# NVIDIA/flowtron

Measured on NVIDIA B200. Metric: training mel-frames/sec, higher is better.
Workload: dtype f16 tensor-core operands (loss-scaled in backward), f32 accumulate+state

## Files before the change

### flowtron_b200/_lib.py

```python
from __future__ import annotations

import ctypes
import os
from ctypes import POINTER, Structure, byref, c_char_p, c_double, c_float, c_int, c_longlong, c_size_t, c_void_p

import torch

_HERE = os.path.dirname(os.path.abspath(__file__))
LIB_PATH = os.path.join(_HERE, "libflowtron_b200.so")

FT_F16, FT_BF16, FT_TF32 = 0, 1, 2
_FMT = {torch.float16: FT_F16, torch.bfloat16: FT_BF16, torch.float32: FT_TF32}

_lib = None


class FtArStepDesc(Structure):
    _fields_ = [("T", c_int), ("B", c_int), ("L", c_int), ("n_mel", c_int), ("n_hidden", c_int), ("n_attn", c_int),
                ("n_text", c_int), ("reversed", c_int), ("has_gate", c_int), ("has_prior", c_int),
                ("temperature", c_float)]


AR_WEIGHT_FIELDS = ["attn_lstm_w_ih", "attn_lstm_w_hh", "attn_lstm_b_ih", "attn_lstm_b_hh",
                    "lstm_w_ih0", "lstm_w_hh0", "lstm_b_ih0", "lstm_b_hh0",
# ... 166 lines not shown


def timing_report():
    buf = ctypes.create_string_buffer(1 << 16)
    lib().ft_timing_report.argtypes = [c_char_p, c_int]
    n = lib().ft_timing_report(buf, len(buf))
    out = []
    for line in buf.raw[:n].decode().splitlines():
        name, m, nn, k, cnt, ms = line.split()
        out.append((name, int(m), int(nn), int(k), int(cnt), float(ms)))
    return out


def _need_cuda(*ts):
    for t in ts:
        if t is not None and not t.is_cuda:
            raise FlowtronB200Error("flowtron_b200 kernels need CUDA tensors (no CPU fallback exists)")


def set_gemm_pair_mode(mode: int):
    lib().ft_set_gemm_pair_mode(int(mode))


def gemm(A, B, *, a_mn=False, b_mn=False, bias=None, bias2=None, act=0, beta=0, alpha=1.0,
         out32=None, out16=None):
    _need_cuda(A, B)
    if a_mn:
        K, M = A.shape
    else:
        M, K = A.shape
    if b_mn:
        Kb, N = B.shape
    else:
        N, Kb = B.shape
    assert K == Kb, (A.shape, B.shape)
    assert A.stride(-1) == 1 and B.stride(-1) == 1
    c16_fmt = 0
    if out16 is not None:
        c16_fmt = _FMT[out16.dtype]
    check(lib().ft_gemm(M, N, K, ptr(A), A.stride(0), _FMT[A.dtype], int(a_mn), ptr(B), B.stride(0), _FMT[B.dtype],
                        int(b_mn), ptr(bias), ptr(bias2), act, beta, float(alpha),
                        ptr(out32), 0 if out32 is None else out32.stride(0),
                        ptr(out16), 0 if out16 is None else out16.stride(0), c16_fmt, stream_ptr()), "ft_gemm")


def lstm_fwd(xproj, whh16, lens, hseq16, gates16=None, cstate=None, h32=None):
# ... 251 lines not shown
```

### flowtron_b200/csrc/api.cu

```cuda
#include <mutex>
#include <string>
#include <atomic>
#include <cstdio>
#include <vector>
#include <map>
#include <tuple>

#include "ft_internal.h"
#include "../../include/flowtron_b200.h"

namespace ft {

static thread_local std::string g_err;
static std::atomic<long long> g_launches{0};
static int* g_status_dev = nullptr;
static std::mutex g_mu;

int ft_set_error(const char* msg) {
    g_err = msg ? msg : "unknown error";
    return -1;
}
int ft_check_launch(const char* what) {
    cudaError_t e = cudaGetLastError();
    if (e != cudaSuccess) {
// ... 75 lines not shown
    }
    return off;
}

long long ft_launch_count(void) { return ft::g_launches.load(); }
void ft_reset_launch_count(void) { ft::g_launches.store(0); }

int ft_gemm(int M, int N, int K, const void* A, long long lda, int a_fmt, int a_mn, const void* B, long long ldb,
            int b_fmt, int b_mn, const float* bias, const float* bias2, int act, int beta, float alpha, float* C32,
            long long ldc32, void* C16, long long ldc16, int c16_fmt, void* stream) {
    ft::GemmArgs g;
    g.M = M; g.N = N; g.K = K;
    g.A = A; g.lda = lda; g.a_fmt = a_fmt; g.a_mn = a_mn;
    g.B = B; g.ldb = ldb; g.b_fmt = b_fmt; g.b_mn = b_mn;
    g.bias = bias; g.bias2 = bias2; g.act = act; g.beta = beta; g.alpha = alpha;
    g.C32 = C32; g.ldc32 = ldc32; g.C16 = C16; g.ldc16 = ldc16; g.c16_fmt = c16_fmt;
    return ft::launch_gemm(g, static_cast<cudaStream_t>(stream));
}

void ft_debug_set_lstm_trace(long long* buf) { ft::set_lstm_trace(buf); }

void ft_set_lstm_half_sm(int on) { ft::set_lstm_half_sm(on); }
void ft_set_gemm_pair_mode(int mode) { ft::set_gemm_pair_mode(mode); }

int ft_lstm_fwd(int T, int B, const float* xproj, const void* whh16, const int* lens, void* hseq16, long long ldh,
                void* gates16, float* cstate, float* h32, long long ldh32, int* flags, void* stream) {
    return ft::launch_lstm_fwd(T, B, xproj, whh16, lens, hseq16, ldh, gates16, cstate, h32, ldh32, flags,
                               static_cast<cudaStream_t>(stream));
}

int ft_lstm_bwd(int T, int B, const float* dh_ext, long long ldd, const void* whhT16, const void* gates16,
                const float* cstate, const int* lens, void* dG16, int* flags, void* stream) {
    return ft::launch_lstm_bwd(T, B, dh_ext, ldd, whhT16, gates16, cstate, lens, dG16, flags,
                               static_cast<cudaStream_t>(stream));
}

}
```

### flowtron_b200/csrc/ar_step.cu

```cuda
#include <cstdlib>
#include <cstring>
#include <map>
#include <mutex>
#include <string>
#include <vector>

#include "ft_internal.h"
#include "../../include/flowtron_b200.h"

namespace ft {

namespace {

constexpr int H = 1024, G = 4096;

struct Region { const char* name; size_t off, bytes; };

struct Plan {
    uint8_t* base = nullptr;
    size_t off = 0;
    std::vector<Region>* regs = nullptr;
    template <typename T>
    T* get(const char* name, size_t n) {
        const size_t bytes = n * sizeof(T);
// ... 220 lines not shown
static Pipe* get_pipe(cudaStream_t main) {
    std::lock_guard<std::mutex> lk(g_side_mu);
    auto it = g_pipes.find(main);
    if (it != g_pipes.end()) return &it->second;
    Pipe pp;
    int prio_lo = 0, prio_hi = 0;
    cudaDeviceGetStreamPriorityRange(&prio_lo, &prio_hi);
    const int pr = pipe_prio() ? prio_hi : prio_lo;
    if (cudaStreamCreateWithPriority(&pp.sA, cudaStreamNonBlocking, pr) != cudaSuccess) return nullptr;
    if (cudaStreamCreateWithPriority(&pp.sB, cudaStreamNonBlocking, pr) != cudaSuccess) return nullptr;
    const int mid = pipe_prio() && prio_hi < prio_lo - 1 ? prio_lo - 1 : prio_lo;
    if (cudaStreamCreateWithPriority(&pp.sC, cudaStreamNonBlocking, mid) != cudaSuccess) return nullptr;
    if (cudaStreamCreateWithPriority(&pp.sD, cudaStreamNonBlocking, prio_lo) != cudaSuccess) return nullptr;
    cudaEventCreateWithFlags(&pp.evJ, cudaEventDisableTiming);
    cudaEventCreateWithFlags(&pp.evD, cudaEventDisableTiming);
    cudaEventCreateWithFlags(&pp.evA, cudaEventDisableTiming);
    cudaEventCreateWithFlags(&pp.evG, cudaEventDisableTiming);
    cudaEventCreateWithFlags(&pp.evB, cudaEventDisableTiming);
    cudaEventCreateWithFlags(&pp.ev0, cudaEventDisableTiming);
    g_pipes[main] = pp;
    return &g_pipes[main];
}

int zero(void* p, size_t bytes, cudaStream_t st) {
    return cudaMemsetAsync(p, 0, bytes, st) == cudaSuccess ? 0 : ft_set_error("cudaMemsetAsync failed");
}
int copy_f32(float* dst, const float* src, size_t n, cudaStream_t st) {
    return cudaMemcpyAsync(dst, src, n * sizeof(float), cudaMemcpyDeviceToDevice, st) == cudaSuccess ? 0 : ft_set_error("cudaMemcpyAsync failed");
}

}

static thread_local cudaEvent_t g_text_ready = nullptr;
void set_text_ready_event(void* ev) { g_text_ready = static_cast<cudaEvent_t>(ev); }

int ar_step_fwd(const FtArStepDesc& d, const FtArStepWeights& w, const float* mel, const float* text, const int* in_lens,
                const int* out_lens, const float* prior, float* mel_out, float* log_s, float* gates, float* attn,
                float* logprob, void* saved, void* scratch, cudaStream_t st) {
    cudaEvent_t text_ready = g_text_ready;
    g_text_ready = nullptr;
    FT_TRY(check_desc(d));
    if (d.has_prior && !prior) return ft_set_error("ar_step_fwd: has_prior set but attn_prior is NULL");
    if (d.has_gate && (!gates || !w.gate_w)) return ft_set_error("ar_step_fwd: has_gate set but gate pointers are NULL");
    const Dims n(d);
    Plan ps; ps.base = static_cast<uint8_t*>(saved);
    Saved S; S.plan(ps, d);
// ... 37 lines not shown
    auto kv_projections = [&](cudaStream_t s2) -> int {
        if (text_ready) {
            if (cudaStreamWaitEvent(s2, text_ready, 0) != cudaSuccess) return ft_set_error("ar_step_fwd: cudaStreamWaitEvent(text_ready) failed");
        }
        FT_TRY(launch_cast(text, 2, S.text16, 0, n.RL * n.E, s2));
        FT_TRY(gemm_fwd(s2, n.RL, n.A, n.E, S.text16, n.E, F.w.wk, n.E, nullptr, nullptr, 0, S.Kp, n.A, nullptr, 0));
        FT_TRY(gemm_fwd(s2, n.RL, n.A, n.E, S.text16, n.E, F.w.wv, n.E, nullptr, nullptr, 0, S.Vp, n.A, nullptr, 0));
        return 0;
    };
    if (pa) {
        const int CH = att_chunk;
        auto xa = [&](cudaStream_t s2, int t0, int t1) {
            const long long r0 = static_cast<long long>(t0) * n.B, rows = static_cast<long long>(t1 - t0) * n.B;
            return gemm_fwd(s2, rows, G, n.M, S.mel_in16 + r0 * n.M, n.M, F.w.w_ih_a, n.M, w.attn_lstm_b_ih, w.attn_lstm_b_hh, 0,
                            F.X1 + r0 * G, G, nullptr, 0);
        };
        cudaStream_t sr = pipe_prio() ? pa->sA : st;
        cudaEventRecord(pa->ev0, st);
        if (sr != st) cudaStreamWaitEvent(sr, pa->ev0, 0);
        cudaStreamWaitEvent(pa->sB, pa->ev0, 0);
        cudaStreamWaitEvent(pa->sC, pa->ev0, 0);
        FT_TRY(kv_projections(pa->sC));
        FT_TRY(xa(sr, 0, CH < n.T ? CH : n.T));
        for (int t0 = 0; t0 < n.T; t0 += CH) {
            const int t1 = t0 + CH < n.T ? t0 + CH : n.T;
            if (t1 < n.T) {
                FT_TRY(xa(pa->sB, t1, t1 + CH < n.T ? t1 + CH : n.T));
                cudaEventRecord(pa->evB, pa->sB);
            }
            FT_TRY(launch_lstm_fwd_chunk(n.T, n.B, t0, t1, F.X1, F.w.w_hh_a, out_lens, S.d16, n.D, S.gatesA, S.cA, F.flags, sr, F.hA32, H));
            cudaEventRecord(pa->evA, sr);
            if (t1 < n.T) cudaStreamWaitEvent(sr, pa->evB, 0);
            cudaStreamWaitEvent(pa->sC, pa->evA, 0);
            FT_TRY(attention_rows(pa->sC, t0, t1));
            const long long r0 = static_cast<long long>(t0) * n.B, rows = static_cast<long long>(t1 - t0) * n.B;
            FT_TRY(gemm_fwd(pa->sC, rows, G, n.D, S.d16 + r0 * n.D, n.D, F.w.w_ih0, n.D, w.lstm_b_ih0, w.lstm_b_hh0, 0, F.X + r0 * G, G, nullptr, 0));
        }
        cudaEventRecord(pa->evG, pa->sC);
        cudaStreamWaitEvent(st, pa->evG, 0);
        if (sr != st) { cudaEventRecord(pa->evJ, sr); cudaStreamWaitEvent(st, pa->evJ, 0); }
        xproj0_done = true;
    } else {
    static int xin = -1;
    if (xin < 0) { const char* e = getenv("FT_LSTM_XIN"); xin = (!e || atoi(e) != 0) ? 1 : 0; }
    if (xin && n.M <= 128 && n.B <= 32) {
        FT_TRY(launch_lstm_fwd_xin(n.T, n.B, S.mel_in16, n.M, n.M, F.w.w_ih_a, w.attn_lstm_b_ih, w.attn_lstm_b_hh, F.w.w_hh_a, out_lens,
                                   S.d16, n.D, S.gatesA, S.cA, F.hA32, H, F.flags, st));
    } else {
        FT_TRY(gemm_fwd(st, n.R, G, n.M, S.mel_in16, n.M, F.w.w_ih_a, n.M, w.attn_lstm_b_ih, w.attn_lstm_b_hh, 0, F.X, G, nullptr, 0));
        FT_TRY(launch_lstm_fwd(n.T, n.B, F.X, F.w.w_hh_a, out_lens, S.d16, n.D, S.gatesA, S.cA, F.hA32, H, F.flags, st));
    }
    FT_TRY(kv_projections(st));
    FT_TRY(attention_rows(st, 0, n.T));
    }

    Pipe* pp = (F.X1 && n.B <= 32 && n.T > pipe_chunk_steps()) ? get_pipe(st) : nullptr;
    if (pp) {
        const int S_ = pipe_chunk_steps();
        int* flagsA = F.flags;
        int* flagsB = F.flags + static_cast<size_t>(S_) * 16;
        if (!xproj0_done) FT_TRY(gemm_fwd(st, n.R, G, n.D, S.d16, n.D, F.w.w_ih0, n.D, w.lstm_b_ih0, w.lstm_b_hh0, 0, F.X, G, nullptr, 0));
        cudaStream_t sr = pipe_prio() ? pp->sA : st;
        cudaEventRecord(pp->ev0, st);
        if (sr != st) cudaStreamWaitEvent(sr, pp->ev0, 0);
        cudaStreamWaitEvent(pp->sB, pp->ev0, 0);
        cudaStreamWaitEvent(pp->sC, pp->ev0, 0);
        for (int t0 = 0; t0 < n.T; t0 += S_) {
            const int t1 = t0 + S_ < n.T ? t0 + S_ : n.T;
            const long long r0 = static_cast<long long>(t0) * n.B, rows = static_cast<long long>(t1 - t0) * n.B;
            FT_TRY(launch_lstm_fwd_chunk(n.T, n.B, t0, t1, F.X, F.w.w_hh0, out_lens, S.h0_16, H, S.gates0, S.c0, flagsA, sr));
            cudaEventRecord(pp->evA, sr);
            cudaStreamWaitEvent(pp->sC, pp->evA, 0);
            FT_TRY(gemm_fwd(pp->sC, rows, G, H, S.h0_16 + r0 * H, H, F.w.w_ih1, H, w.lstm_b_ih1, w.lstm_b_hh1, 0,
                            F.X1 + r0 * G, G, nullptr, 0));
            cudaEventRecord(pp->evG, pp->sC);
            cudaStreamWaitEvent(pp->sB, pp->evG, 0);
            FT_TRY(launch_lstm_fwd_chunk(n.T, n.B, t0, t1, F.X1, F.w.w_hh1, out_lens, S.h1_16, H, S.gates1, S.c1, flagsB, pp->sB));
        }
        cudaEventRecord(pp->evB, pp->sB);
        cudaStreamWaitEvent(st, pp->evB, 0);
        if (sr != st) { cudaEventRecord(pp->evJ, sr); cudaStreamWaitEvent(st, pp->evJ, 0); }
    } else {
        if (!xproj0_done) FT_TRY(gemm_fwd(st, n.R, G, n.D, S.d16, n.D, F.w.w_ih0, n.D, w.lstm_b_ih0, w.lstm_b_hh0, 0, F.X, G, nullptr, 0));
        FT_TRY(launch_lstm_fwd(n.T, n.B, F.X, F.w.w_hh0, out_lens, S.h0_16, H, S.gates0, S.c0, nullptr, 0, F.flags, st));
        FT_TRY(gemm_fwd(st, n.R, G, H, S.h0_16, H, F.w.w_ih1, H, w.lstm_b_ih1, w.lstm_b_hh1, 0, F.X, G, nullptr, 0));
        FT_TRY(launch_lstm_fwd(n.T, n.B, F.X, F.w.w_hh1, out_lens, S.h1_16, H, S.gates1, S.c1, nullptr, 0, F.flags, st));
    }

    FT_TRY(gemm_fwd(st, n.R, H, H, S.h1_16, H, F.w.w1, H, w.dense_b0, nullptr, 1, nullptr, 0, S.y1_16, H));
// ... 77 lines not shown
        a.in_lens = in_lens; a.out_lens = out_lens; a.attn = attn; a.p_save = S_.p_save; a.temperature = d.temperature;
        a.dctx = C.dd + H; a.lddc = n.D; a.dattn_ext = d_attn; a.dlp_ext = d_logprob; a.scale = S;
        a.dQ = F.dQ; a.lddq = n.A; a.dK = F.dK; a.lddk = n.A; a.dV = F.dV; a.lddv = n.A; a.dv = g.att_v;
        a.t_begin = t0; a.t_end = t1;
        FT_TRY(launch_attn_bwd(a, s2));
        FT_TRY(launch_cast(F.dQ + r0 * n.A, 2, F.dQ16 + r0 * n.A, 0, rows * n.A, s2));
        FT_TRY(gemm_dgrad(s2, rows, H, n.A, F.dQ16 + r0 * n.A, n.A, F.w.wq, H, 1, C.dd + r0 * n.D, n.D, nullptr, 0, nullptr, 0));
        return 0;
    };
    static int attb_pipe = -1;
    if (attb_pipe < 0) { const char* e = getenv("FT_ATTB_PIPE"); attb_pipe = e ? atoi(e) : 0; }
    bool attention_bwd_done = false;
    Pipe* pp = (F.dcarry1 && n.B <= 32 && 2 * pipe_chunk_steps() <= n.T) ? get_pipe(st) : nullptr;
    if (pp) {
        const int S_c = pipe_chunk_steps();
        int* flagsA = F.flags;
        int* flagsB = F.flags + static_cast<size_t>(S_c) * 64;
        cudaStream_t sr = pipe_prio() ? pp->sA : st;
        cudaEventRecord(pp->ev0, st);
        if (sr != st) cudaStreamWaitEvent(sr, pp->ev0, 0);
        cudaStreamWaitEvent(pp->sB, pp->ev0, 0);
        cudaStreamWaitEvent(pp->sC, pp->ev0, 0);
        const int n_chunks = (n.T + S_c - 1) / S_c;
        for (int c = n_chunks - 1; c >= 0; --c) {
            const int t0 = c * S_c, t1 = t0 + S_c < n.T ? t0 + S_c : n.T;
            const long long r0 = static_cast<long long>(t0) * n.B, rows = static_cast<long long>(t1 - t0) * n.B;
            FT_TRY(launch_lstm_bwd_chunk(n.T, n.B, t0, t1, F.dh, H, F.w.w_hh1, S_.gates1, S_.c1, out_lens, F.dG1, F.dcarry1, flagsA, sr));
            cudaEventRecord(pp->evA, sr);
            cudaStreamWaitEvent(pp->sC, pp->evA, 0);
            FT_TRY(gemm_dgrad(pp->sC, rows, H, G, F.dG1 + r0 * G, G, F.w.w_ih1, H, 0, F.dh + r0 * H, H, nullptr, 0, nullptr, 0));
            cudaEventRecord(pp->evG, pp->sC);
            cudaStreamWaitEvent(pp->sB, pp->evG, 0);
            FT_TRY(launch_lstm_bwd_chunk(n.T, n.B, t0, t1, F.dh, H, F.w.w_hh0, S_.gates0, S_.c0, out_lens, F.dG0, F.dcarry0, flagsB, pp->sB));
            if (attb_pipe && S_c % 64 == 0) {
                if (c == n_chunks - 1) cudaStreamWaitEvent(pp->sD, pp->ev0, 0);
                cudaEventRecord(pp->evD, pp->sB);
                cudaStreamWaitEvent(pp->sD, pp->evD, 0);
                FT_TRY(attention_bwd_rows(pp->sD, t0, t1));
                attention_bwd_done = true;
            }
        }
        if (attention_bwd_done) { cudaEventRecord(pp->evD, pp->sD); cudaStreamWaitEvent(st, pp->evD, 0); }
        if (sr != st) { cudaEventRecord(pp->evJ, sr); cudaStreamWaitEvent(st, pp->evJ, 0); }
        ss = fork_side(sd, st);
        FT_TRY(gemm_wgrad(ss, G, H, Rm, F.dG1 + static_cast<size_t>(n.B) * G, G, S_.h1_16, H, g.lstm_w_hh1, H, iS));
        FT_TRY(gemm_wgrad(ss, G, H, R, F.dG1, G, S_.h0_16, H, g.lstm_w_ih1, H, iS));
        FT_TRY(launch_colsum(F.dG1, 0, G, R, G, g.lstm_b_ih1, iS, ss));
        FT_TRY(copy_f32(g.lstm_b_hh1, g.lstm_b_ih1, G, ss));
        cudaEventRecord(pp->evB, pp->sB);
        cudaStreamWaitEvent(st, pp->evB, 0);
    } else {
    FT_TRY(launch_lstm_bwd(n.T, n.B, F.dh, H, F.w.w_hh1, S_.gates1, S_.c1, out_lens, F.dG1, F.flags, st));
    ss = fork_side(sd, st);
    FT_TRY(gemm_wgrad(ss, G, H, Rm, F.dG1 + static_cast<size_t>(n.B) * G, G, S_.h1_16, H, g.lstm_w_hh1, H, iS));
    FT_TRY(gemm_wgrad(ss, G, H, R, F.dG1, G, S_.h0_16, H, g.lstm_w_ih1, H, iS));
    FT_TRY(launch_colsum(F.dG1, 0, G, R, G, g.lstm_b_ih1, iS, ss));
    FT_TRY(copy_f32(g.lstm_b_hh1, g.lstm_b_ih1, G, ss));
    FT_TRY(gemm_dgrad(st, R, H, G, F.dG1, G, F.w.w_ih1, H, 0, F.dh, H, nullptr, 0, nullptr, 0));

    FT_TRY(launch_lstm_bwd(n.T, n.B, F.dh, H, F.w.w_hh0, S_.gates0, S_.c0, out_lens, F.dG0, F.flags, st));
    }
    static int attb_chunk = -1;
    if (attb_chunk < 0) { const char* e = getenv("FT_ATT_OVERLAP_BWD"); attb_chunk = e ? atoi(e) : 256; if (attb_chunk % 64) attb_chunk = 0; }
    Pipe* pq = (may_fuse_bptt && !attention_bwd_done && attb_chunk > 0 && F.dcarry1 && n.B <= 32 && n.T >= attb_chunk + 64) ? get_pipe(st) : nullptr;
    if (pq) {
        FT_TRY(launch_cast(w.attn_lstm_w_ih, 2, F.w.w_ih_a, 0, static_cast<long long>(G) * n.M, st));
        FT_TRY(launch_transpose_cast_f16(w.attn_lstm_w_hh, F.w.w_hh_a, G, H, st));
        cudaStream_t sr = pipe_prio() ? pq->sA : st;
        cudaEventRecord(pq->ev0, st);
        if (sr != st) cudaStreamWaitEvent(sr, pq->ev0, 0);
        cudaStreamWaitEvent(pq->sC, pq->ev0, 0);
        const int CH = attb_chunk, n_chunks = (n.T + CH - 1) / CH;
        for (int c = n_chunks - 1; c >= 0; --c) {
            const int t0 = c * CH, t1 = t0 + CH < n.T ? t0 + CH : n.T;
            FT_TRY(attention_bwd_rows(pq->sC, t0, t1));
            cudaEventRecord(pq->evG, pq->sC);
            cudaStreamWaitEvent(sr, pq->evG, 0);
            FT_TRY(launch_lstm_bwd_chunk(n.T, n.B, t0, t1, C.dd, n.D, F.w.w_hh_a, S_.gatesA, S_.cA, out_lens, F.dGa, F.dcarry1, F.flags, sr));
        }
        cudaStreamWaitEvent(st, pq->evG, 0);
        if (sr != st) { cudaEventRecord(pq->evJ, sr); cudaStreamWaitEvent(st, pq->evJ, 0); }
        if (bptt_done) *bptt_done = true;
    } else if (!attention_bwd_done) {
        FT_TRY(attention_bwd_rows(st, 0, n.T));
    }

    FT_TRY(launch_cast(F.dK, 2, F.dK16, 0, RL * n.A, st));
    FT_TRY(launch_cast(F.dV, 2, F.dV16, 0, RL * n.A, st));
    FT_TRY(gemm_dgrad(st, RL, n.E, n.A, F.dK16, n.A, F.w.wk, n.E, 0, d_text, n.E, nullptr, 0, nullptr, 0, iS));
    FT_TRY(gemm_dgrad(st, RL, n.E, n.A, F.dV16, n.A, F.w.wv, n.E, 1, d_text, n.E, nullptr, 0, nullptr, 0, iS));

    join_side(sd, st);
    return 0;
}

// ... 122 lines not shown
```

### flowtron_b200/csrc/attention.cu

```cuda
#include "ptx.cuh"
#include "ft_internal.h"

namespace ft {

constexpr int AT_TT = 64;
constexpr int AT_LB = 128;
constexpr int AT_AC = 64;
constexpr int AT_THREADS = 256;
constexpr int SQ_LD = AT_TT + 4;
constexpr int SK_LD = AT_LB + 4;

struct AttnFwdParams {
    int t_begin, t_end;
    int T, B, L, A;
    const float* Q; long long ldq;
    const float* K; long long ldk;
    const float* V; long long ldv;
    const float* v;
    const int* in_lens;
    const int* out_lens;
    const float* prior;
    int reversed;
    float inv_temperature;
    float* attn; float* logprob;
// ... 507 lines not shown
                        if (j < ns && ac + aa < p.A && x != 0.f)
                            atomicAdd(p.dK + (static_cast<long long>(l0 + s0 + j) * p.B + b) * p.lddk + ac + aa, x * 4.f * sv[ac + aa]);
                    }
                }
            }
            if (a_ok) {
                const float s4 = 4.f * sv[ac + a_l];
#pragma unroll
                for (int i = 0; i < 16; ++i) {
                    const int tt = grp * 16 + i;
                    if (tt < nrows) p.dQ[(static_cast<long long>(t0 + tt) * p.B + b) * p.lddq + ac + a_l] = dq[i] * s4;
                }
                atomicAdd(&sdv[ac + a_l], (grp == 0 ? sumde : 0.f) - 2.f * dvr);
            }
        }
    }
    __syncthreads();
    for (int i = tid; i < p.A; i += AT_THREADS) {
        const float x = sdv[i];
        if (x != 0.f) atomicAdd(p.dv + i, x * iS);
    }
}

static size_t attn_fwd_smem(int L, int A) {
    const int Lr = (L + 31) & ~31;
    return sizeof(float) * (static_cast<size_t>(AT_AC) * SQ_LD + AT_AC * SK_LD + AT_TT * (Lr + 4) + A) + 64;
}
static size_t attn_bwd_smem(int L, int A) {
    const int Lr = (L + 31) & ~31;
    return sizeof(float) * (static_cast<size_t>(AT_AC) * SQ_LD + AT_AC * SK_LD + AT_TT * (Lr + 4) + 2 * A) + 64;
}

int launch_attn_fwd(const AttnFwdArgs& a, cudaStream_t st) {
    if (a.L > 512) return ft_set_error("attention: L > 512 not supported");
    if (a.A % 4) return ft_set_error("attention: A must be a multiple of 4");
    AttnFwdParams p;
    p.T = a.T; p.B = a.B; p.L = a.L; p.A = a.A;
    p.Q = a.Q; p.ldq = a.ldq; p.K = a.K; p.ldk = a.ldk; p.V = a.V; p.ldv = a.ldv; p.v = a.v;
    p.in_lens = a.in_lens; p.out_lens = a.out_lens; p.prior = a.prior; p.reversed = a.reversed;
    p.inv_temperature = 1.0f / a.temperature;
    p.attn = a.attn; p.logprob = a.logprob; p.p_save = a.p_save;
    p.ctx16 = static_cast<__half*>(a.ctx16); p.ldc = a.ldc; p.ctx32 = a.ctx32; p.ldc32 = a.ldc32;
    const size_t smem = attn_fwd_smem(a.L, a.A);
    cudaFuncSetAttribute(attn_fwd_kernel, cudaFuncAttributeMaxDynamicSharedMemorySize, static_cast<int>(smem));
    p.t_begin = a.t_begin; p.t_end = a.t_end > 0 ? a.t_end : a.T;
    if (p.t_begin % AT_TT || p.t_begin < 0 || p.t_end > a.T || p.t_end <= p.t_begin) return ft_set_error("attention: bad query range");
    dim3 grid((p.t_end - p.t_begin + AT_TT - 1) / AT_TT, a.B);
    TimeScope ts("attn_fwd", p.t_end - p.t_begin, a.B, a.L, st);
    attn_fwd_kernel<<<grid, AT_THREADS, smem, st>>>(p);
    ft_count_launch(1);
    return ft_check_launch("attn_fwd_kernel");
}

int launch_attn_bwd(const AttnBwdArgs& a, cudaStream_t st) {
    if (a.L > 256) return ft_set_error("attention backward: L > 256 not supported");
    AttnBwdParams p;
    p.T = a.T; p.B = a.B; p.L = a.L; p.A = a.A;
    p.Q = a.Q; p.ldq = a.ldq; p.K = a.K; p.ldk = a.ldk; p.V = a.V; p.ldv = a.ldv; p.v = a.v;
    p.in_lens = a.in_lens; p.out_lens = a.out_lens; p.attn = a.attn; p.p_save = a.p_save;
    p.has_prior = a.p_save != nullptr; p.inv_temperature = 1.0f / a.temperature;
    p.dctx = a.dctx; p.lddc = a.lddc; p.dattn_ext = a.dattn_ext; p.dlp_ext = a.dlp_ext; p.scale = a.scale;
    p.dQ = a.dQ; p.lddq = a.lddq; p.dK = a.dK; p.lddk = a.lddk; p.dV = a.dV; p.lddv = a.lddv; p.dv = a.dv;
    const size_t smem = attn_bwd_smem(a.L, a.A);
    cudaFuncSetAttribute(attn_bwd_kernel, cudaFuncAttributeMaxDynamicSharedMemorySize, static_cast<int>(smem));
    p.t_begin = a.t_begin; p.t_end = a.t_end > 0 ? a.t_end : a.T;
    if (p.t_begin % AT_TT || p.t_begin < 0 || p.t_end > a.T || p.t_end <= p.t_begin) return ft_set_error("attention backward: bad query range");
    dim3 grid((p.t_end - p.t_begin + AT_TT - 1) / AT_TT, a.B);
    TimeScope ts("attn_bwd", p.t_end - p.t_begin, a.B, a.L, st);
    attn_bwd_kernel<<<grid, AT_THREADS, smem, st>>>(p);
    ft_count_launch(1);
    return ft_check_launch("attn_bwd_kernel");
}

}
```

### flowtron_b200/csrc/elementwise.cu

```cuda
#include "ptx.cuh"
#include "ft_internal.h"

namespace ft {

static int num_sms() {
    static int n = 0;
    if (!n) {
        int dev = 0;
        cudaGetDevice(&dev);
        cudaDeviceGetAttribute(&n, cudaDevAttrMultiProcessorCount, dev);
    }
    return n;
}
static inline int grid_for(long long work_items, int threads, int per_sm = 8) {
    long long blocks = (work_items + threads - 1) / threads;
    long long cap = static_cast<long long>(num_sms()) * per_sm;
    return static_cast<int>(blocks < 1 ? 1 : (blocks > cap ? cap : blocks));
}

__device__ __forceinline__ int back_index_d(int t, int len, int T) { return t < len ? len - 1 - t : T - 1 - t + len; }

template <typename TO>
__device__ __forceinline__ TO cvt_from_float(float x);
template <> __device__ __forceinline__ __half cvt_from_float<__half>(float x) { return __float2half_rn(fminf(fmaxf(x, -65504.f), 65504.f)); }
template <> __device__ __forceinline__ __nv_bfloat16 cvt_from_float<__nv_bfloat16>(float x) { return __float2bfloat16_rn(x); }
template <> __device__ __forceinline__ float cvt_from_float<float>(float x) { return x; }
__device__ __forceinline__ float cvt_to_float(float x) { return x; }
__device__ __forceinline__ float cvt_to_float(__half x) { return __half2float(x); }
__device__ __forceinline__ float cvt_to_float(__nv_bfloat16 x) { return __bfloat162float(x); }

template <typename TI, typename TO>
__global__ void cast_kernel(const TI* __restrict__ src, TO* __restrict__ dst, long long n) {
    const long long stride = static_cast<long long>(gridDim.x) * blockDim.x * 4;
    for (long long i = (static_cast<long long>(blockIdx.x) * blockDim.x + threadIdx.x) * 4; i < n; i += stride) {
        if (i + 3 < n) {
            TO o[4];
#pragma unroll
            for (int j = 0; j < 4; ++j) o[j] = cvt_from_float<TO>(cvt_to_float(src[i + j]));
#pragma unroll
// ... 187 lines not shown
        const float g = dgate[r];
        if (g == 0.f) continue;
        db += g;
        const __half* drow = d16 + r * ldd;
        float* ddrow = dd + r * lddd;
#pragma unroll
        for (int j = 0; j < GB_KJ; ++j) {
            const int k = threadIdx.x + 256 * j;
            if (k < K) {
                acc[j] = fmaf(g, __half2float(drow[k]), acc[j]);
                ddrow[k] = fmaf(g, w[j], ddrow[k]);
            }
        }
    }
    if (threadIdx.x == 0 && db != 0.f) atomicAdd(dbg, db);
#pragma unroll
    for (int j = 0; j < GB_KJ; ++j) {
        const int k = threadIdx.x + 256 * j;
        if (k < K && acc[j] != 0.f) atomicAdd(dwg + k, acc[j]);
    }
}
int launch_gate_bwd(const void* d16, long long ldd, int K, const float* wg, const float* dgate, long long R, float* dd,
                    long long lddd, float* dwg, float* dbg, const float* scale, cudaStream_t st) {
    long long gl = (R + 15) / 16, gcap = static_cast<long long>(num_sms()) * 4;
    int g = static_cast<int>(gl > gcap ? gcap : gl);
    if (g < 1) g = 1;
    if (K > 2048) return ft_set_error("gate_bwd: K > 2048 not supported");
    gate_bwd_kernel<<<g, 256, 0, st>>>(static_cast<const __half*>(d16), ldd, K, wg, dgate, R, dd, lddd, dwg, dbg, scale);
    ft_count_launch(1);
    return ft_check_launch("gate_bwd_kernel");
}

__global__ void affine_fwd_kernel(const float* __restrict__ o, const float* __restrict__ mel_flow, const int* __restrict__ lens,
                                  int T, int B, int M, int reversed, float* __restrict__ z, float* __restrict__ log_s) {
    const long long n = static_cast<long long>(T) * B * M;
    for (long long i = static_cast<long long>(blockIdx.x) * blockDim.x + threadIdx.x; i < n;
         i += static_cast<long long>(gridDim.x) * blockDim.x) {
        const int m = static_cast<int>(i % M);
        const long long rb = i / M;
        const int b = static_cast<int>(rb % B), q = static_cast<int>(rb / B);
        const float ls = o[rb * 2 * M + m], bb = o[rb * 2 * M + M + m];
        log_s[i] = ls;
        const float zz = expf(ls) * mel_flow[i] + bb;
        int s = q;
        if (reversed) s = back_index_d(q, lens ? lens[b] : T, T);
        z[(static_cast<long long>(s) * B + b) * M + m] = zz;
    }
// ... 192 lines not shown
```

### flowtron_b200/csrc/ft_internal.h

```cpp
#pragma once
#include <cuda.h>
#include <cuda_runtime.h>
#include <stdint.h>

namespace ft {

typedef CUresult (*PFN_encodeTiled)(CUtensorMap*, CUtensorMapDataType, cuuint32_t, void*, const cuuint64_t*,
                                    const cuuint64_t*, const cuuint32_t*, const cuuint32_t*, CUtensorMapInterleave,
                                    CUtensorMapSwizzle, CUtensorMapL2promotion, CUtensorMapFloatOOBfill);

int ft_set_error(const char* msg);
int ft_check_launch(const char* what);
int* ft_status_word();
void ft_count_launch(int n);

struct TimeScope {
    TimeScope(const char* name, long long m, long long n, long long k, cudaStream_t st);
    ~TimeScope();
    cudaStream_t st_; int idx_;
};

enum { FMT_F16 = 0, FMT_BF16 = 1, FMT_TF32 = 2 };

struct GemmArgs {
    int M = 0, N = 0, K = 0;
    const void* A = nullptr; long long lda = 0; int a_fmt = 0; int a_mn = 0;
    const void* B = nullptr; long long ldb = 0; int b_fmt = 0; int b_mn = 0;
    const float* bias = nullptr; const float* bias2 = nullptr;
    int act = 0; int beta = 0; float alpha = 1.0f; const float* alpha_ptr = nullptr;
    const void* aux16 = nullptr; long long ldaux = 0;
    float* C32 = nullptr; long long ldc32 = 0;
    void* C16 = nullptr; long long ldc16 = 0; int c16_fmt = 0;
};
int launch_gemm(const GemmArgs& g, cudaStream_t st);
void set_gemm_pair_mode(int mode);
int make_tmap_2d(CUtensorMap* out, const void* ptr, int fmt, long long rows, long long cols, long long ld,
                 int box_cols, int box_rows);

void set_lstm_trace(long long* p);
void set_lstm_half_sm(int on);
int launch_lstm_fwd(int T, int B, const float* xproj, const void* whh16, const int* lens, void* hseq16, long long ldh,
                    void* gates16, float* cstate, float* h32, long long ldh32, int* flags, cudaStream_t st);
int launch_lstm_fwd_xin(int T, int B, const void* x16, long long ldx, int kx, const void* wih16, const float* b_ih, const float* b_hh,
                        const void* whh16, const int* lens, void* hseq16, long long ldh, void* gates16, float* cstate, float* h32,
                        long long ldh32, int* flags, cudaStream_t st);
int launch_lstm_fwd_chunk(int T, int B, int t0, int t1, const float* xproj, const void* whh16, const int* lens, void* hseq16,
                          long long ldh, void* gates16, float* cstate, int* flags, cudaStream_t st, float* h32 = nullptr,
                          long long ldh32 = 0);
int launch_lstm_bwd_chunk(int T, int B, int t0, int t1, const float* dh_ext, long long ldd, const void* whhT16, const void* gates16,
                          const float* cstate, const int* lens, void* dG16, float* dc_carry, int* flags, cudaStream_t st);
int launch_lstm_bwd(int T, int B, const float* dh_ext, long long ldd, const void* whhT16, const void* gates16,
                    const float* cstate, const int* lens, void* dG16, int* flags, cudaStream_t st);

int launch_cast(const void* src, int src_fmt, void* dst, int dst_fmt, long long n, cudaStream_t st);
int launch_transpose_cast_f16(const float* src, void* dst, int rows, int cols, cudaStream_t st);
int launch_grad_scale(const float* a, long long na, const float* b, long long nb, const float* c, long long nc, float target,
                      float* scale2, cudaStream_t st, const float* d = nullptr, long long nd = 0, const float* e = nullptr,
                      long long ne = 0);
// ... 40 lines not shown
```

### flowtron_b200/csrc/gemm.cu

```cuda
#include <cstdlib>

#include "ptx.cuh"
#include "ft_internal.h"

namespace ft {

constexpr int BM = 128;
constexpr int TILE_BYTES = BM * 128;

struct GemmParams {
    int M, N, K;
    int a_fmt, b_fmt;
    int a_mn, b_mn;
    const float* bias;
    const float* bias2;
    int act;
    const __half* aux16; long long ldaux;
    int beta;
    float alpha;
    const float* alpha_ptr;
    float* C32; long long ldc32;
    void* C16; long long ldc16; int c16_fmt;
    int* status;
    int tma_out = 0;
// ... 329 lines not shown
PFN_encodeTiled get_tma_encoder() { return ensure_tma_encoder() ? nullptr : g_encode; }

int make_tmap_2d(CUtensorMap* out, const void* ptr, int fmt, long long rows, long long cols, long long ld,
                 int box_cols, int box_rows) {
    if (ensure_tma_encoder()) return -1;
    const int elt = (fmt == 2) ? 4 : 2;
    CUtensorMapDataType dt = fmt == 0 ? CU_TENSOR_MAP_DATA_TYPE_FLOAT16
                           : fmt == 1 ? CU_TENSOR_MAP_DATA_TYPE_BFLOAT16 : CU_TENSOR_MAP_DATA_TYPE_FLOAT32;
    if ((reinterpret_cast<uintptr_t>(ptr) & 15) || ((ld * elt) & 15)) return ft_set_error("TMA operand must be 16-byte aligned with a 16-byte-multiple row pitch");
    if (box_cols * elt != 128) return ft_set_error("TMA box inner extent must be 128 bytes (SWIZZLE_128B)");
    cuuint64_t dims[2] = {static_cast<cuuint64_t>(cols), static_cast<cuuint64_t>(rows)};
    cuuint64_t strides[1] = {static_cast<cuuint64_t>(ld * elt)};
    cuuint32_t box[2] = {static_cast<cuuint32_t>(box_cols), static_cast<cuuint32_t>(box_rows)};
    cuuint32_t estr[2] = {1, 1};
    CUresult r = g_encode(out, dt, 2, const_cast<void*>(ptr), dims, strides, box, estr, CU_TENSOR_MAP_INTERLEAVE_NONE,
                          CU_TENSOR_MAP_SWIZZLE_128B, CU_TENSOR_MAP_L2_PROMOTION_L2_256B,
                          CU_TENSOR_MAP_FLOAT_OOB_FILL_NONE);
    if (r != CUDA_SUCCESS) return ft_set_error("cuTensorMapEncodeTiled failed");
    return 0;
}

static int g_pair_mode = -1;
void set_gemm_pair_mode(int mode) { g_pair_mode = mode; }

int launch_gemm(const GemmArgs& g, cudaStream_t st) {
    if (g.M <= 0 || g.N <= 0 || g.K <= 0) return 0;
    const bool tf32 = (g.a_fmt == 2);
    if ((g.a_fmt == 2) != (g.b_fmt == 2)) return ft_set_error("gemm: tf32 must be used for both operands");
    if (tf32 && (g.a_mn || g.b_mn)) return ft_set_error("gemm: MN-major tf32 operands not supported");
    const int elt = tf32 ? 4 : 2, BK = 128 / elt;
    CUtensorMap tmA, tmB;
    int rc;
    if (!g.a_mn) rc = make_tmap_2d(&tmA, g.A, g.a_fmt, g.M, g.K, g.lda, BK, BM);
    else         rc = make_tmap_2d(&tmA, g.A, g.a_fmt, g.K, g.M, g.lda, BK, BK);
    if (rc) return rc;
    if (!g.b_mn) rc = make_tmap_2d(&tmB, g.B, g.b_fmt, g.N, g.K, g.ldb, BK, 128);
    else         rc = make_tmap_2d(&tmB, g.B, g.b_fmt, g.K, g.N, g.ldb, BK, BK);
    if (rc) return rc;
    GemmParams p;
    p.M = g.M; p.N = g.N; p.K = g.K; p.a_fmt = g.a_fmt; p.b_fmt = g.b_fmt; p.a_mn = g.a_mn; p.b_mn = g.b_mn;
    p.bias = g.bias; p.bias2 = g.bias2; p.act = g.act; p.alpha_ptr = g.alpha_ptr; p.aux16 = static_cast<const __half*>(g.aux16); p.ldaux = g.ldaux; p.beta = g.beta; p.alpha = g.alpha;
    p.C32 = g.C32; p.ldc32 = g.ldc32; p.C16 = g.C16; p.ldc16 = g.ldc16; p.c16_fmt = g.c16_fmt;
    p.status = ft_status_word();
    CUtensorMap tmC = tmA;
    {
        static int tma_env = -1;
        if (tma_env < 0) { const char* e = getenv("FT_GEMM_TMA_STORE"); tma_env = (!e || atoi(e) != 0) ? 1 : 0; }
        const bool one = (g.C32 != nullptr) != (g.C16 != nullptr);
        const bool plain = !g.beta && (g.N % 4 == 0) && (!g.bias || (reinterpret_cast<uintptr_t>(g.bias) & 15) == 0) &&
                           (!g.bias2 || (reinterpret_cast<uintptr_t>(g.bias2) & 15) == 0) &&
                           (g.act != 2 || (((reinterpret_cast<uintptr_t>(g.aux16) & 7) == 0) && (g.ldaux % 4 == 0)));
        if (tma_env && one && plain) {
            const void* cp = g.C32 ? static_cast<const void*>(g.C32) : g.C16;
            const long long ldc = g.C32 ? g.ldc32 : g.ldc16;
            const int elt_c = g.C32 ? 4 : 2;
            if ((reinterpret_cast<uintptr_t>(cp) & 15) == 0 && ((ldc * elt_c) & 15) == 0) {
                const int fmt_c = g.C32 ? 2 : g.c16_fmt;
                if (make_tmap_2d(&tmC, cp, fmt_c, g.M, g.N, ldc, 128 / elt_c, 32)) return -1;
                p.tma_out = g.C32 ? 1 : 2;
            }
        }
    }
    { static int dbg = -1; if (dbg < 0) { const char* e = getenv("FT_GEMM_EPI_DEBUG"); dbg = e ? atoi(e) : 0; } p.dbg = dbg; }
    {
        static int sms = 0;
        if (!sms) { int dev = 0; cudaGetDevice(&dev); cudaDeviceGetAttribute(&sms, cudaDevAttrMultiProcessorCount, dev); }
        bool wide = (g.N % 256 == 0) || g.N > 1024;
        if (wide && static_cast<long long>((g.N + 255) / 256) * ((g.M + BM - 1) / BM) < sms) wide = false;
        const int bn = wide ? 256 : 128;
        const int tiles_n = (g.N + bn - 1) / bn, tiles_m = (g.M + BM - 1) / BM;
        const long long n_tiles_ll = static_cast<long long>(tiles_n) * tiles_m;
        if (n_tiles_ll > 0x7fffffff) return ft_set_error("gemm: too many tiles");
        const int n_tiles = static_cast<int>(n_tiles_ll);
        const int num_kb_all = (g.K + BK - 1) / BK;
        int splitk = 1;
        const bool splittable = g.C32 && !g.C16 && !g.beta && !g.bias && !g.bias2 && g.act == 0 && (g.N % 4 == 0) &&
                                g.ldc32 == g.N && ((reinterpret_cast<uintptr_t>(g.C32) & 15) == 0);
        if (splittable && n_tiles * 2 <= sms && num_kb_all >= 64) {
            splitk = sms / n_tiles;
            if (splitk > 16) splitk = 16;
            while (splitk > 1 && num_kb_all / splitk < 16) --splitk;
        }
        if (splitk > 1) p.tma_out = 0;
        if (splitk > 1) {
            if (cudaMemsetAsync(g.C32, 0, sizeof(float) * static_cast<size_t>(g.M) * g.N, st) != cudaSuccess) return ft_set_error("gemm: memset failed");
        }
        p.splitk = splitk;
        if (g_pair_mode < 0) { const char* e = getenv("FT_GEMM_2CTA"); g_pair_mode = e ? atoi(e) : 1; }
        const long long tiles_m2 = (g.M + 2 * BM - 1) / (2 * BM);
        const bool big = 2.0 * g.M * g.N * g.K >= 1e11;
        if ((g_pair_mode == 2 || (g_pair_mode == 1 && big)) && wide && splitk == 1 && tiles_m2 * tiles_n >= sms / 2) {
            const int n_tiles2 = static_cast<int>(tiles_m2 * tiles_n);
            const int n_pairs = n_tiles2 < sms / 2 ? n_tiles2 : sms / 2;
            if (!g.b_mn) { if (make_tmap_2d(&tmB, g.B, g.b_fmt, g.N, g.K, g.ldb, BK, 128)) return -1; }
            static bool attr_pair = false;
            if (!attr_pair) {
                cudaFuncSetAttribute(gemm2_kernel<false, 256, 2>, cudaFuncAttributeMaxDynamicSharedMemorySize, G2Cfg<256, 2>::SMEM);
                cudaFuncSetAttribute(gemm2_kernel<true, 256, 2>, cudaFuncAttributeMaxDynamicSharedMemorySize, G2Cfg<256, 2>::SMEM);
                attr_pair = true;
            }
            cudaLaunchConfig_t cfg = {};
            cfg.gridDim = dim3(2 * n_pairs); cfg.blockDim = dim3(G2_THREADS); cfg.dynamicSmemBytes = G2Cfg<256, 2>::SMEM; cfg.stream = st;
            cudaLaunchAttribute attr[1];
            attr[0].id = cudaLaunchAttributeClusterDimension;
            attr[0].val.clusterDim.x = 2; attr[0].val.clusterDim.y = 1; attr[0].val.clusterDim.z = 1;
            cfg.attrs = attr; cfg.numAttrs = 1;
            TimeScope ts(g.a_mn ? "gemm_wgrad" : (g.b_mn ? "gemm_dgrad" : "gemm_fwd"), g.M, g.N, g.K, st);
            cudaError_t e = tf32 ? cudaLaunchKernelEx(&cfg, gemm2_kernel<true, 256, 2>, tmA, tmB, tmC, p, tiles_n, n_tiles2)
                                 : cudaLaunchKernelEx(&cfg, gemm2_kernel<false, 256, 2>, tmA, tmB, tmC, p, tiles_n, n_tiles2);
            if (e != cudaSuccess) return ft_set_error(cudaGetErrorString(e));
            ft_count_launch(1);
            return ft_check_launch("gemm2_kernel<pair>");
        }
        const long long n_work = static_cast<long long>(n_tiles) * splitk;
        const int grid2 = n_work < sms ? static_cast<int>(n_work) : sms;
        if (!g.b_mn && bn == 256) { if (make_tmap_2d(&tmB, g.B, g.b_fmt, g.N, g.K, g.ldb, BK, 256)) return -1; }
        static bool attr2 = false;
        if (!attr2) {
            cudaFuncSetAttribute(gemm2_kernel<false, 256>, cudaFuncAttributeMaxDynamicSharedMemorySize, G2Cfg<256>::SMEM);
            cudaFuncSetAttribute(gemm2_kernel<false, 128>, cudaFuncAttributeMaxDynamicSharedMemorySize, G2Cfg<128>::SMEM);
            cudaFuncSetAttribute(gemm2_kernel<true, 256>, cudaFuncAttributeMaxDynamicSharedMemorySize, G2Cfg<256>::SMEM);
            cudaFuncSetAttribute(gemm2_kernel<true, 128>, cudaFuncAttributeMaxDynamicSharedMemorySize, G2Cfg<128>::SMEM);
            attr2 = true;
        }
        TimeScope ts(g.a_mn ? "gemm_wgrad" : (g.b_mn ? "gemm_dgrad" : "gemm_fwd"), g.M, g.N, g.K, st);
        if (tf32) {
            if (wide) gemm2_kernel<true, 256><<<grid2, G2_THREADS, G2Cfg<256>::SMEM, st>>>(tmA, tmB, tmC, p, tiles_n, n_tiles);
            else      gemm2_kernel<true, 128><<<grid2, G2_THREADS, G2Cfg<128>::SMEM, st>>>(tmA, tmB, tmC, p, tiles_n, n_tiles);
        } else {
            if (wide) gemm2_kernel<false, 256><<<grid2, G2_THREADS, G2Cfg<256>::SMEM, st>>>(tmA, tmB, tmC, p, tiles_n, n_tiles);
            else      gemm2_kernel<false, 128><<<grid2, G2_THREADS, G2Cfg<128>::SMEM, st>>>(tmA, tmB, tmC, p, tiles_n, n_tiles);
        }
        ft_count_launch(1);
        return ft_check_launch("gemm2_kernel");
    }
}

}
// ... 1 lines not shown
```

### include/flowtron_b200.h

```cpp
#ifndef FLOWTRON_B200_H
#define FLOWTRON_B200_H
#include <stddef.h>
#include <stdint.h>

#ifdef __cplusplus
extern "C" {
#endif

#define FT_F16 0
#define FT_BF16 1
#define FT_TF32 2

int ft_version(void);
const char* ft_last_error(void);
int ft_device_status(void);
void ft_timing_enable(int on);
void ft_timing_reset(void);
int ft_timing_report(char* buf, int cap);
long long ft_launch_count(void);
void ft_reset_launch_count(void);

int ft_gemm(int M, int N, int K, const void* A, long long lda, int a_fmt, int a_mn, const void* B, long long ldb,
            int b_fmt, int b_mn, const float* bias, const float* bias2, int act, int beta, float alpha, float* C32,
            long long ldc32, void* C16, long long ldc16, int c16_fmt, void* stream);

int ft_lstm_fwd(int T, int B, const float* xproj, const void* whh16, const int* lens, void* hseq16, long long ldh,
                void* gates16, float* cstate, float* h32, long long ldh32, int* flags, void* stream);

void ft_debug_set_lstm_trace(long long* buf);
void ft_debug_set_infer_trace(long long* buf);

void ft_set_lstm_half_sm(int on);
void ft_set_gemm_pair_mode(int mode);

int ft_lstm_bwd(int T, int B, const float* dh_ext, long long ldd, const void* whhT16, const void* gates16,
                const float* cstate, const int* lens, void* dG16, int* flags, void* stream);

typedef struct {
    int T, B, L;
    int n_mel;
    int n_hidden;
    int n_attn;
    int n_text;
    int reversed;
    int has_gate;
    int has_prior;
    float temperature;
} FtArStepDesc;

typedef struct {
    float *attn_lstm_w_ih, *attn_lstm_w_hh, *attn_lstm_b_ih, *attn_lstm_b_hh;
    float *lstm_w_ih0, *lstm_w_hh0, *lstm_b_ih0, *lstm_b_hh0;
    float *lstm_w_ih1, *lstm_w_hh1, *lstm_b_ih1, *lstm_b_hh1;
    float *att_query, *att_key, *att_value, *att_v;
    float *dense_w0, *dense_b0, *dense_w1, *dense_b1;
    float *conv_w, *conv_b;
// ... 112 lines not shown
```

Baseline: 520,000.

## Cap side-stream kernel grids to leave SMs for concurrent LSTM recurrences

Adds a thread-local SM budget and applies it as an RAII scope around the chunked loops that run alongside persistent LSTM recurrence kernels, assuming each recurrence holds 64 CTAs. Persistent GEMM grids, elementwise grid caps and 2-CTA pair counts use the budget in place of the full SM count. Attention forward and backward launches are split into several smaller launches sized to fit the budget. The aim is to stop side-stream work from occupying SMs the recurrences need, so they can overlap instead of serialising, at the cost of more launches and less parallelism for the side work.

Result: no change. 523,900 (median of 6 runs) (+0.8%).

```diff
diff --git a/flowtron_b200/_lib.py b/flowtron_b200/_lib.py
--- a/flowtron_b200/_lib.py
+++ b/flowtron_b200/_lib.py
@@ -212,6 +212,10 @@
     lib().ft_set_gemm_pair_mode(int(mode))
 
 
+def set_sm_budget(sms: int):
+    lib().ft_set_sm_budget(int(sms))
+
+
 def gemm(A, B, *, a_mn=False, b_mn=False, bias=None, bias2=None, act=0, beta=0, alpha=1.0,
          out32=None, out16=None):
     _need_cuda(A, B)
diff --git a/flowtron_b200/csrc/api.cu b/flowtron_b200/csrc/api.cu
--- a/flowtron_b200/csrc/api.cu
+++ b/flowtron_b200/csrc/api.cu
@@ -121,6 +121,7 @@
 
 void ft_set_lstm_half_sm(int on) { ft::set_lstm_half_sm(on); }
 void ft_set_gemm_pair_mode(int mode) { ft::set_gemm_pair_mode(mode); }
+void ft_set_sm_budget(int sms) { ft::set_sm_budget(sms); }
 
 int ft_lstm_fwd(int T, int B, const float* xproj, const void* whh16, const int* lens, void* hseq16, long long ldh,
                 void* gates16, float* cstate, float* h32, long long ldh32, int* flags, void* stream) {
diff --git a/flowtron_b200/csrc/ar_step.cu b/flowtron_b200/csrc/ar_step.cu
--- a/flowtron_b200/csrc/ar_step.cu
+++ b/flowtron_b200/csrc/ar_step.cu
@@ -266,6 +266,16 @@
     return &g_pipes[main];
 }
 
+struct SmBudget {
+    static constexpr int kRecurrenceCtas = 64;
+    const int prev;
+    explicit SmBudget(int recurrences) : prev(sm_budget()) {
+        const int free_sms = device_sms() - recurrences * kRecurrenceCtas;
+        set_sm_budget(prev > 0 && prev < free_sms ? prev : free_sms);
+    }
+    ~SmBudget() { set_sm_budget(prev); }
+};
+
 int zero(void* p, size_t bytes, cudaStream_t st) {
     return cudaMemsetAsync(p, 0, bytes, st) == cudaSuccess ? 0 : ft_set_error("cudaMemsetAsync failed");
 }
@@ -349,6 +359,8 @@
         cudaStreamWaitEvent(pa->sC, pa->ev0, 0);
         FT_TRY(kv_projections(pa->sC));
         FT_TRY(xa(sr, 0, CH < n.T ? CH : n.T));
+        {
+        SmBudget budget(1);
         for (int t0 = 0; t0 < n.T; t0 += CH) {
             const int t1 = t0 + CH < n.T ? t0 + CH : n.T;
             if (t1 < n.T) {
@@ -363,6 +375,7 @@
             const long long r0 = static_cast<long long>(t0) * n.B, rows = static_cast<long long>(t1 - t0) * n.B;
             FT_TRY(gemm_fwd(pa->sC, rows, G, n.D, S.d16 + r0 * n.D, n.D, F.w.w_ih0, n.D, w.lstm_b_ih0, w.lstm_b_hh0, 0, F.X + r0 * G, G, nullptr, 0));
         }
+        }
         cudaEventRecord(pa->evG, pa->sC);
         cudaStreamWaitEvent(st, pa->evG, 0);
         if (sr != st) { cudaEventRecord(pa->evJ, sr); cudaStreamWaitEvent(st, pa->evJ, 0); }
@@ -392,6 +405,7 @@
         if (sr != st) cudaStreamWaitEvent(sr, pp->ev0, 0);
         cudaStreamWaitEvent(pp->sB, pp->ev0, 0);
         cudaStreamWaitEvent(pp->sC, pp->ev0, 0);
+        SmBudget budget(2);
         for (int t0 = 0; t0 < n.T; t0 += S_) {
             const int t1 = t0 + S_ < n.T ? t0 + S_ : n.T;
             const long long r0 = static_cast<long long>(t0) * n.B, rows = static_cast<long long>(t1 - t0) * n.B;
@@ -515,6 +529,8 @@
         cudaStreamWaitEvent(pp->sB, pp->ev0, 0);
         cudaStreamWaitEvent(pp->sC, pp->ev0, 0);
         const int n_chunks = (n.T + S_c - 1) / S_c;
+        {
+        SmBudget budget(2);
         for (int c = n_chunks - 1; c >= 0; --c) {
             const int t0 = c * S_c, t1 = t0 + S_c < n.T ? t0 + S_c : n.T;
             const long long r0 = static_cast<long long>(t0) * n.B, rows = static_cast<long long>(t1 - t0) * n.B;
@@ -533,6 +549,7 @@
                 attention_bwd_done = true;
             }
         }
+        }
         if (attention_bwd_done) { cudaEventRecord(pp->evD, pp->sD); cudaStreamWaitEvent(st, pp->evD, 0); }
         if (sr != st) { cudaEventRecord(pp->evJ, sr); cudaStreamWaitEvent(st, pp->evJ, 0); }
         ss = fork_side(sd, st);
@@ -564,6 +581,7 @@
         if (sr != st) cudaStreamWaitEvent(sr, pq->ev0, 0);
         cudaStreamWaitEvent(pq->sC, pq->ev0, 0);
         const int CH = attb_chunk, n_chunks = (n.T + CH - 1) / CH;
+        SmBudget budget(1);
         for (int c = n_chunks - 1; c >= 0; --c) {
             const int t0 = c * CH, t1 = t0 + CH < n.T ? t0 + CH : n.T;
             FT_TRY(attention_bwd_rows(pq->sC, t0, t1));
diff --git a/flowtron_b200/csrc/attention.cu b/flowtron_b200/csrc/attention.cu
--- a/flowtron_b200/csrc/attention.cu
+++ b/flowtron_b200/csrc/attention.cu
@@ -553,6 +553,13 @@
     }
 }
 
+static int rows_per_launch(const void* fn, size_t smem, int B, int rows) {
+    if (sm_budget() <= 0) return rows;
+    int occ = 0;
+    if (cudaOccupancyMaxActiveBlocksPerMultiprocessor(&occ, fn, AT_THREADS, smem) != cudaSuccess || occ < 1) occ = 1;
+    const int tiles = occ * launch_sms() / B;
+    return tiles < 1 ? AT_TT : tiles * AT_TT;
+}
 static size_t attn_fwd_smem(int L, int A) {
     const int Lr = (L + 31) & ~31;
     return sizeof(float) * (static_cast<size_t>(AT_AC) * SQ_LD + AT_AC * SK_LD + AT_TT * (Lr + 4) + A) + 64;
@@ -576,11 +583,17 @@
     cudaFuncSetAttribute(attn_fwd_kernel, cudaFuncAttributeMaxDynamicSharedMemorySize, static_cast<int>(smem));
     p.t_begin = a.t_begin; p.t_end = a.t_end > 0 ? a.t_end : a.T;
     if (p.t_begin % AT_TT || p.t_begin < 0 || p.t_end > a.T || p.t_end <= p.t_begin) return ft_set_error("attention: bad query range");
-    dim3 grid((p.t_end - p.t_begin + AT_TT - 1) / AT_TT, a.B);
-    TimeScope ts("attn_fwd", p.t_end - p.t_begin, a.B, a.L, st);
-    attn_fwd_kernel<<<grid, AT_THREADS, smem, st>>>(p);
-    ft_count_launch(1);
-    return ft_check_launch("attn_fwd_kernel");
+    const int t_begin = p.t_begin, t_end = p.t_end;
+    const int step = rows_per_launch(reinterpret_cast<const void*>(attn_fwd_kernel), smem, a.B, t_end - t_begin);
+    for (p.t_begin = t_begin; p.t_begin < t_end; p.t_begin += step) {
+        p.t_end = t_end - p.t_begin > step ? p.t_begin + step : t_end;
+        dim3 grid((p.t_end - p.t_begin + AT_TT - 1) / AT_TT, a.B);
+        TimeScope ts("attn_fwd", p.t_end - p.t_begin, a.B, a.L, st);
+        attn_fwd_kernel<<<grid, AT_THREADS, smem, st>>>(p);
+        ft_count_launch(1);
+        if (ft_check_launch("attn_fwd_kernel")) return -1;
+    }
+    return 0;
 }
 
 int launch_attn_bwd(const AttnBwdArgs& a, cudaStream_t st) {
@@ -596,11 +609,17 @@
     cudaFuncSetAttribute(attn_bwd_kernel, cudaFuncAttributeMaxDynamicSharedMemorySize, static_cast<int>(smem));
     p.t_begin = a.t_begin; p.t_end = a.t_end > 0 ? a.t_end : a.T;
     if (p.t_begin % AT_TT || p.t_begin < 0 || p.t_end > a.T || p.t_end <= p.t_begin) return ft_set_error("attention backward: bad query range");
-    dim3 grid((p.t_end - p.t_begin + AT_TT - 1) / AT_TT, a.B);
-    TimeScope ts("attn_bwd", p.t_end - p.t_begin, a.B, a.L, st);
-    attn_bwd_kernel<<<grid, AT_THREADS, smem, st>>>(p);
-    ft_count_launch(1);
-    return ft_check_launch("attn_bwd_kernel");
-}
-
-}
+    const int t_begin = p.t_begin, t_end = p.t_end;
+    const int step = rows_per_launch(reinterpret_cast<const void*>(attn_bwd_kernel), smem, a.B, t_end - t_begin);
+    for (p.t_begin = t_begin; p.t_begin < t_end; p.t_begin += step) {
+        p.t_end = t_end - p.t_begin > step ? p.t_begin + step : t_end;
+        dim3 grid((p.t_end - p.t_begin + AT_TT - 1) / AT_TT, a.B);
+        TimeScope ts("attn_bwd", p.t_end - p.t_begin, a.B, a.L, st);
+        attn_bwd_kernel<<<grid, AT_THREADS, smem, st>>>(p);
+        ft_count_launch(1);
+        if (ft_check_launch("attn_bwd_kernel")) return -1;
+    }
+    return 0;
+}
+
+}
diff --git a/flowtron_b200/csrc/elementwise.cu b/flowtron_b200/csrc/elementwise.cu
--- a/flowtron_b200/csrc/elementwise.cu
+++ b/flowtron_b200/csrc/elementwise.cu
@@ -3,18 +3,9 @@
 
 namespace ft {
 
-static int num_sms() {
-    static int n = 0;
-    if (!n) {
-        int dev = 0;
-        cudaGetDevice(&dev);
-        cudaDeviceGetAttribute(&n, cudaDevAttrMultiProcessorCount, dev);
-    }
-    return n;
-}
 static inline int grid_for(long long work_items, int threads, int per_sm = 8) {
     long long blocks = (work_items + threads - 1) / threads;
-    long long cap = static_cast<long long>(num_sms()) * per_sm;
+    long long cap = static_cast<long long>(launch_sms()) * per_sm;
     return static_cast<int>(blocks < 1 ? 1 : (blocks > cap ? cap : blocks));
 }
 
@@ -248,7 +239,7 @@
 }
 int launch_gate_bwd(const void* d16, long long ldd, int K, const float* wg, const float* dgate, long long R, float* dd,
                     long long lddd, float* dwg, float* dbg, const float* scale, cudaStream_t st) {
-    long long gl = (R + 15) / 16, gcap = static_cast<long long>(num_sms()) * 4;
+    long long gl = (R + 15) / 16, gcap = static_cast<long long>(launch_sms()) * 4;
     int g = static_cast<int>(gl > gcap ? gcap : gl);
     if (g < 1) g = 1;
     if (K > 2048) return ft_set_error("gate_bwd: K > 2048 not supported");
diff --git a/flowtron_b200/csrc/ft_internal.h b/flowtron_b200/csrc/ft_internal.h
--- a/flowtron_b200/csrc/ft_internal.h
+++ b/flowtron_b200/csrc/ft_internal.h
@@ -34,6 +34,11 @@
 };
 int launch_gemm(const GemmArgs& g, cudaStream_t st);
 void set_gemm_pair_mode(int mode);
+
+void set_sm_budget(int sms);
+int sm_budget();
+int device_sms();
+int launch_sms();
 int make_tmap_2d(CUtensorMap* out, const void* ptr, int fmt, long long rows, long long cols, long long ld,
                  int box_cols, int box_rows);
 
diff --git a/flowtron_b200/csrc/gemm.cu b/flowtron_b200/csrc/gemm.cu
--- a/flowtron_b200/csrc/gemm.cu
+++ b/flowtron_b200/csrc/gemm.cu
@@ -375,6 +375,16 @@
 
 static int g_pair_mode = -1;
 void set_gemm_pair_mode(int mode) { g_pair_mode = mode; }
+
+static thread_local int g_sm_budget = 0;
+void set_sm_budget(int sms) { g_sm_budget = sms > 0 ? sms : 0; }
+int sm_budget() { return g_sm_budget; }
+int device_sms() {
+    static int n = 0;
+    if (!n) { int dev = 0; cudaGetDevice(&dev); cudaDeviceGetAttribute(&n, cudaDevAttrMultiProcessorCount, dev); }
+    return n;
+}
+int launch_sms() { const int n = device_sms(); return g_sm_budget > 0 && g_sm_budget < n ? g_sm_budget : n; }
 
 int launch_gemm(const GemmArgs& g, cudaStream_t st) {
     if (g.M <= 0 || g.N <= 0 || g.K <= 0) return 0;
@@ -416,8 +426,7 @@
     }
     { static int dbg = -1; if (dbg < 0) { const char* e = getenv("FT_GEMM_EPI_DEBUG"); dbg = e ? atoi(e) : 0; } p.dbg = dbg; }
     {
-        static int sms = 0;
-        if (!sms) { int dev = 0; cudaGetDevice(&dev); cudaDeviceGetAttribute(&sms, cudaDevAttrMultiProcessorCount, dev); }
+        const int sms = device_sms(), grid_sms = launch_sms();
         bool wide = (g.N % 256 == 0) || g.N > 1024;
         if (wide && static_cast<long long>((g.N + 255) / 256) * ((g.M + BM - 1) / BM) < sms) wide = false;
         const int bn = wide ? 256 : 128;
@@ -442,9 +451,9 @@
         if (g_pair_mode < 0) { const char* e = getenv("FT_GEMM_2CTA"); g_pair_mode = e ? atoi(e) : 1; }
         const long long tiles_m2 = (g.M + 2 * BM - 1) / (2 * BM);
         const bool big = 2.0 * g.M * g.N * g.K >= 1e11;
-        if ((g_pair_mode == 2 || (g_pair_mode == 1 && big)) && wide && splitk == 1 && tiles_m2 * tiles_n >= sms / 2) {
+        if ((g_pair_mode == 2 || (g_pair_mode == 1 && big)) && wide && splitk == 1 && grid_sms >= 2 && tiles_m2 * tiles_n >= sms / 2) {
             const int n_tiles2 = static_cast<int>(tiles_m2 * tiles_n);
-            const int n_pairs = n_tiles2 < sms / 2 ? n_tiles2 : sms / 2;
+            const int n_pairs = n_tiles2 < grid_sms / 2 ? n_tiles2 : grid_sms / 2;
             if (!g.b_mn) { if (make_tmap_2d(&tmB, g.B, g.b_fmt, g.N, g.K, g.ldb, BK, 128)) return -1; }
             static bool attr_pair = false;
             if (!attr_pair) {
@@ -466,7 +475,7 @@
             return ft_check_launch("gemm2_kernel<pair>");
         }
         const long long n_work = static_cast<long long>(n_tiles) * splitk;
-        const int grid2 = n_work < sms ? static_cast<int>(n_work) : sms;
+        const int grid2 = n_work < grid_sms ? static_cast<int>(n_work) : grid_sms;
         if (!g.b_mn && bn == 256) { if (make_tmap_2d(&tmB, g.B, g.b_fmt, g.N, g.K, g.ldb, BK, 256)) return -1; }
         static bool attr2 = false;
         if (!attr2) {
diff --git a/include/flowtron_b200.h b/include/flowtron_b200.h
--- a/include/flowtron_b200.h
+++ b/include/flowtron_b200.h
@@ -32,6 +32,7 @@
 
 void ft_set_lstm_half_sm(int on);
 void ft_set_gemm_pair_mode(int mode);
+void ft_set_sm_budget(int sms);
 
 int ft_lstm_bwd(int T, int B, const float* dh_ext, long long ldd, const void* whhT16, const void* gates16,
                 const float* cstate, const int* lens, void* dG16, int* flags, void* stream);
```
